# tinganchen/AlignQ

Hardware: AMD Instinct MI355X
Metric: images/sec (train step, CDF+ADMM) ResNet-20 8-bit (higher is better)
Workload: dtype f32; 1 GPU; resnet20 CIFAR-shape 3x32x32, 8W/8A CDF+ADMM full train step (cdf_alignment_admm/resnet-20-cifar-10), batch 128/GPU, HIP-graph replay, batch-norm folded into the site kernels, channels-last tensors, all Conv2d_Q convolutions on alignq_conv*_nhwc (exact-product bf16 MFMA); global_batch=128, parallelism=dp1

## Files before the change

alignq_amd/csrc/conv_kernels.hip:

```cpp
#include <hip/hip_runtime.h>
#include <stdint.h>
#include <stdlib.h>

#include "../../include/alignq.h"
#include "site_internal.h"
#include "store_forms.h"
#include "wgrad_reduce_body.h"

namespace {

using namespace alignq_wgr;

typedef __bf16 bf16x8 __attribute__((ext_vector_type(8)));
typedef __bf16 bf16x4 __attribute__((ext_vector_type(4)));
typedef float f32x4 __attribute__((ext_vector_type(4)));
typedef short s16x4 __attribute__((ext_vector_type(4)));

#ifdef ALIGNQ_STAMPS
__device__ unsigned long long g_conv_stamps[64];
__device__ unsigned long long g_conv_blk[2][4096];
#define STAMP(on, i)                                                          \
  do {                                                                        \
    if ((on) && threadIdx.x == 0) g_conv_stamps[i] = wall_clock64();          \
  } while (0)
// ... 477 lines not shown
  if (bn_part) {
    float* red = reinterpret_cast<float*>(lds);
#define ROW_SHR_ADD(V, CTRL) V += __builtin_bit_cast(float, __builtin_amdgcn_update_dpp(0, __builtin_bit_cast(int, V), CTRL, 0xf, 0xf, false))
#pragma unroll
    for (int e = 0; e < 4; e++) {
      ROW_SHR_ADD(bs[e], 0x111); ROW_SHR_ADD(bs[e], 0x112); ROW_SHR_ADD(bs[e], 0x114); ROW_SHR_ADD(bs[e], 0x118);
      ROW_SHR_ADD(bq[e], 0x111); ROW_SHR_ADD(bq[e], 0x112); ROW_SHR_ADD(bq[e], 0x114); ROW_SHR_ADD(bq[e], 0x118);
    }
#undef ROW_SHR_ADD
    __syncthreads();
    if ((lane & 15) == 15) {
#pragma unroll
      for (int e = 0; e < 4; e++) {
        red[(wv * 16 + 4 * q + e) * 2] = bs[e];
        red[(wv * 16 + 4 * q + e) * 2 + 1] = bq[e];
      }
    }
    __syncthreads();
    if (tid < COUT) {
      const int cg = tid / 16, cl = tid % 16;
      float s0 = 0.f, s1 = 0.f;
#pragma unroll
      for (int ppi = 0; ppi < NPP; ppi++) {
        s0 += red[((ppi * NCG + cg) * 16 + cl) * 2];
        s1 += red[((ppi * NCG + cg) * 16 + cl) * 2 + 1];
      }
      bn_part[((int64_t)tid * n_wg + block) * 2] = s0;
      bn_part[((int64_t)tid * n_wg + block) * 2 + 1] = s1;
    }
  }
}

template <int CIN, int COUT, int WDI, int KS, int S, int PT, bool IMG = false>
__global__ __launch_bounds__(256) void convgen_fwd_kernel(const float* __restrict__ x, const float* __restrict__ w,
                                                          float* __restrict__ y, int H, int total_rows, float nlev,
                                                          float* __restrict__ bn_part) {
  __shared__ __attribute__((aligned(16))) __bf16 lds[3 * ConvGen<CIN, COUT, WDI, KS, S, PT>::ARR];
  convgen_fwd_body<CIN, COUT, WDI, KS, S, PT, IMG>(x, w, y, H, total_rows, nlev, bn_part, lds, blockIdx.x, gridDim.x);
}

template <int CIN, int COUT, int WDI, int PT3, int PT1, bool IMG = false>
__global__ __launch_bounds__(256) void transition_fwd_kernel(const float* __restrict__ x, const float* __restrict__ w3,
                                                             const float* __restrict__ w1, float* __restrict__ y3,
                                                             float* __restrict__ y1, int H, int total_rows, float nlev,
                                                             float* __restrict__ part3, float* __restrict__ part1, int n3) {
  constexpr int A3 = ConvGen<CIN, COUT, WDI, 3, 2, PT3>::ARR, A1 = ConvGen<CIN, COUT, WDI, 1, 2, PT1>::ARR;
  __shared__ __attribute__((aligned(16))) __bf16 lds[3 * (A3 > A1 ? A3 : A1)];
  if ((int)blockIdx.x < n3)
    convgen_fwd_body<CIN, COUT, WDI, 3, 2, PT3, IMG>(x, w3, y3, H, total_rows, nlev, part3, lds, blockIdx.x, n3);
  else
    convgen_fwd_body<CIN, COUT, WDI, 1, 2, PT1, IMG>(x, w1, y1, H, total_rows, nlev, part1, lds, blockIdx.x - n3,
                                                     (int)gridDim.x - n3);
}

template <int CIN, int COUT, int WDI, int KS, int PT, bool WITH1, bool IMG = false>
__device__ __forceinline__ void dgrad_s2_body(const float* __restrict__ dy, const float* __restrict__ w,
                                              float* __restrict__ dx, int H, int total_rows, float nlev,
                                              const float* __restrict__ add, BnLazy lazy, __bf16* lds, int block,
                                              const float* __restrict__ dy1 = nullptr, const float* __restrict__ w1 = nullptr,
                                              BnLazy lazy1 = BnLazy{nullptr, nullptr, nullptr, nullptr}) {
  static_assert(!WITH1 || KS == 3, "the second source is the 1x1 shortcut of a 3x3 transition");
  constexpr int P = KS == 3 ? 1 : 0;
  constexpr int WDO = WDI / 2, TR = PT / WDI;
  constexpr int DROWS = TR / 2 + P, DCOLS = WDO + P;
  constexpr int CP = COUT + 8;
  constexpr int NPIX3 = DROWS * DCOLS + 1;
  constexpr int NPIX1 = WITH1 ? (TR / 2) * WDO : 0;
  constexpr int NPIX = NPIX3 + NPIX1;
  constexpr int ARR = NPIX * CP;
  constexpr int NT = KS * KS + (WITH1 ? 1 : 0);
  constexpr int NS = (NT * COUT + 31) / 32;
  constexpr int NCG = CIN / 16, NPP = 4 / NCG, NG = PT / 16;
  __bf16* Xhi = lds;
  __bf16* Xmi = lds + ARR;
  __bf16* Xlo = lds + 2 * ARR;
  const int tid = threadIdx.x, lane = tid & 63, wv = tid >> 6;
  const int row0 = block * TR;
  const int Ho = H / 2;
  const int orow0 = (row0 / H) * Ho + (row0 % H) / 2;
  const int oimg_hi = (row0 / H + 1) * Ho;
  {
    constexpr int C4 = COUT / 4;
    constexpr int N4 = NPIX3 * C4;
    constexpr int NIT = (N4 + 255) / 256;
    constexpr int M4 = NPIX1 * C4;
    constexpr int NI1 = WITH1 ? (M4 + 255) / 256 : 1;
    float4 v[NIT], zz[NIT], v1[NI1], z1[NI1];
#pragma unroll
    for (int it = 0; it < NIT; it++) {
      const int i = tid + 256 * it;
      const int c4 = i % C4, pix = i / C4;
      const int lr = pix / DCOLS, col = pix % DCOLS;
      const int grow = orow0 + lr;
      const bool ok = i < N4 && pix < DROWS * DCOLS && col < WDO && grow < oimg_hi;
      const int64_t off = ok ? ((int64_t)grow * WDO + col) * COUT + 4 * c4 : 0;
      v[it] = *reinterpret_cast<const float4*>(dy + off);
      if (lazy.z) zz[it] = *reinterpret_cast<const float4*>(lazy.z + off);
      if (!ok) v[it] = make_float4(0.f, 0.f, 0.f, 0.f);
    }
    if constexpr (WITH1) {
#pragma unroll
      for (int it = 0; it < NI1; it++) {
        const int i = tid + 256 * it;
        const int64_t off = i < M4 ? ((int64_t)orow0 * WDO) * COUT + 4 * (int64_t)i : 0;
        v1[it] = *reinterpret_cast<const float4*>(dy1 + off);
        if (lazy1.z) z1[it] = *reinterpret_cast<const float4*>(lazy1.z + off);
      }
    }
    const int c4t = tid % C4;
    if (lazy.z) {
      const float4 a4 = *reinterpret_cast<const float4*>(lazy.ab + 4 * c4t);
      const float4 m4 = *reinterpret_cast<const float4*>(lazy.save + 4 * c4t);
      const float4 i4 = *reinterpret_cast<const float4*>(lazy.save + COUT + 4 * c4t);
      float4 k0, k1;
      if (lazy.part) {
        __shared__ __attribute__((aligned(16))) float kt[2 * COUT];
        bn_totals_lds<COUT>(lazy, kt, block == 0);
        k0 = *reinterpret_cast<const float4*>(kt + 4 * c4t);
        k1 = *reinterpret_cast<const float4*>(kt + COUT + 4 * c4t);
      } else {
        k0 = *reinterpret_cast<const float4*>(lazy.ktot + 4 * c4t);
        k1 = *reinterpret_cast<const float4*>(lazy.ktot + COUT + 4 * c4t);
      }
#pragma unroll
      for (int it = 0; it < NIT; it++) {
        const int i = tid + 256 * it;
        const int pix = i / C4;
        const int lr = pix / DCOLS, col = pix % DCOLS;
        const bool ok = i < N4 && pix < DROWS * DCOLS && col < WDO && orow0 + lr < oimg_hi;
        if (ok) v[it] = bn_lazy4(v[it], zz[it], a4, m4, i4, k0, k1);
      }
    }
    if constexpr (WITH1) {
      if (lazy1.z) {
        const float4 a4 = *reinterpret_cast<const float4*>(lazy1.ab + 4 * c4t);
        const float4 m4 = *reinterpret_cast<const float4*>(lazy1.save + 4 * c4t);
        const float4 i4 = *reinterpret_cast<const float4*>(lazy1.save + COUT + 4 * c4t);
        float4 k0, k1;
        if (lazy1.part) {
          __shared__ __attribute__((aligned(16))) float kt1[2 * COUT];
          bn_totals_lds<COUT>(lazy1, kt1, block == 0);
          k0 = *reinterpret_cast<const float4*>(kt1 + 4 * c4t);
          k1 = *reinterpret_cast<const float4*>(kt1 + COUT + 4 * c4t);
        } else {
          k0 = *reinterpret_cast<const float4*>(lazy1.ktot + 4 * c4t);
          k1 = *reinterpret_cast<const float4*>(lazy1.ktot + COUT + 4 * c4t);
        }
#pragma unroll
        for (int it = 0; it < NI1; it++) {
          if (tid + 256 * it < M4) v1[it] = bn_lazy4(v1[it], z1[it], a4, m4, i4, k0, k1);
        }
      }
    }
#pragma unroll
    for (int it = 0; it < NIT + (WITH1 ? NI1 : 0); it++) {
      const bool second = it >= NIT;
      const int i = tid + 256 * (second ? it - NIT : it);
      if (i < (second ? M4 : N4)) {
        const int c4 = i % C4, pix = (second ? NPIX3 : 0) + i / C4;
        bf16x4 h4, m4, l4;
        const float4 src = second ? v1[second ? it - NIT : 0] : v[second ? 0 : it];
        const float vv[4] = {src.x, src.y, src.z, src.w};
#pragma unroll
        for (int e = 0; e < 4; e++) {
          const __bf16 hi = (__bf16)vv[e];
          const float r1 = vv[e] - (float)hi;
          const __bf16 mi = (__bf16)r1;
          h4[e] = hi; m4[e] = mi; l4[e] = (__bf16)(r1 - (float)mi);
        }
        const int o = pix * CP + 4 * c4;
        *reinterpret_cast<bf16x4*>(Xhi + o) = h4;
        *reinterpret_cast<bf16x4*>(Xmi + o) = m4;
        *reinterpret_cast<bf16x4*>(Xlo + o) = l4;
      }
    }
  }
  const int cig = wv % NCG, pp = wv / NCG;
  const int m = lane & 15, q = lane >> 4;
  bf16x8 ab[NS];
  if constexpr (IMG) {
    static_assert((KS * KS * COUT) % 32 == 0 && COUT % 32 == 0, "whole k steps per filter");
    constexpr int NS3 = KS * KS * COUT / 32;
    const bf16x8* __restrict__ wi = reinterpret_cast<const bf16x8*>(w) + (cig * NS3) * 64 + lane;
#pragma unroll
    for (int s = 0; s < NS3; s++) ab[s] = wi[s * 64];
    if constexpr (WITH1) {
      const bf16x8* __restrict__ wj = reinterpret_cast<const bf16x8*>(w1) + (cig * (NS - NS3)) * 64 + lane;
#pragma unroll
      for (int s = NS3; s < NS; s++) ab[s] = wj[(s - NS3) * 64];
    }
  } else {
#pragma unroll
    for (int s = 0; s < NS; s++) {
      const int k0 = 32 * s + 8 * q;
      const int tap = k0 / COUT, c0 = k0 % COUT;
#pragma unroll
      for (int j = 0; j < 8; j++) {
        float v = 0.f;
        if (tap < KS * KS) v = w[((int64_t)(c0 + j) * (KS * KS) + tap) * CIN + cig * 16 + m];
        else if (WITH1 && tap == KS * KS) v = w1[(int64_t)(c0 + j) * CIN + cig * 16 + m];
        ab[s][j] = (__bf16)rintf(v * nlev);
      }
    }
  }
  __syncthreads();
  for (int g = pp; g < NG; g += NPP) {
    const int p = g * 16 + (lane & 15);
    const int r = p / WDI, c = p % WDI;
    f32x4 acc = {0.f, 0.f, 0.f, 0.f};
#pragma unroll
    for (int s = 0; s < NS; s++) {
      const int k0 = 32 * s + 8 * q;
      const int tap = k0 / COUT, c0 = k0 % COUT;
      int pix = DROWS * DCOLS;
      if (tap < KS * KS) {
        const int ky = tap / KS, kx = tap % KS;
        const int a = r + P - ky, b = c + P - kx;
        if (a >= 0 && b >= 0 && !(a & 1) && !(b & 1)) pix = (a >> 1) * DCOLS + (b >> 1);
      } else if (WITH1 && tap == KS * KS) {
        if (!(r & 1) && !(c & 1)) pix = NPIX3 + (r >> 1) * WDO + (c >> 1);
      }
      const int o = pix * CP + c0;
      const bf16x8 bh = *reinterpret_cast<const bf16x8*>(Xhi + o);
      const bf16x8 bm = *reinterpret_cast<const bf16x8*>(Xmi + o);
      const bf16x8 bl = *reinterpret_cast<const bf16x8*>(Xlo + o);
      acc = __builtin_amdgcn_mfma_f32_16x16x32_bf16(ab[s], bl, acc, 0, 0, 0);
      acc = __builtin_amdgcn_mfma_f32_16x16x32_bf16(ab[s], bm, acc, 0, 0, 0);
      acc = __builtin_amdgcn_mfma_f32_16x16x32_bf16(ab[s], bh, acc, 0, 0, 0);
    }
    const int grow = row0 + r;
    if (grow < total_rows) {
      const int64_t o = ((int64_t)grow * WDI + c) * CIN + cig * 16 + 4 * q;
      float4 out = make_float4(acc[0] / nlev, acc[1] / nlev, acc[2] / nlev, acc[3] / nlev);
      if (add) {
        const float4 a4 = *reinterpret_cast<const float4*>(add + o);
        out.x += a4.x; out.y += a4.y; out.z += a4.z; out.w += a4.w;
      }
      alignq_store::st16<alignq_store::kConvOut>(dx + o, out);
    }
  }
}

template <int CIN, int COUT, int WDI, int KS, int PT, bool WITH1>
struct DgradS2Lds {
  static constexpr int P = KS == 3 ? 1 : 0, TR = PT / WDI;
  static constexpr int kBf16 = 3 * (((TR / 2 + P) * (WDI / 2 + P) + 1) + (WITH1 ? (TR / 2) * (WDI / 2) : 0)) * (COUT + 8);
};

template <int CIN, int COUT, int WDI, int KS, int PT, bool IMG = false>
__global__ __launch_bounds__(256) void dgrad_s2_kernel(const float* __restrict__ dy, const float* __restrict__ w,
                                                       float* __restrict__ dx, int H, int total_rows, float nlev,
                                                       const float* __restrict__ add, BnLazy lazy) {
  __shared__ __attribute__((aligned(16))) __bf16 lds[DgradS2Lds<CIN, COUT, WDI, KS, PT, false>::kBf16];
  dgrad_s2_body<CIN, COUT, WDI, KS, PT, false, IMG>(dy, w, dx, H, total_rows, nlev, add, lazy, lds, blockIdx.x);
}

template <int CIN, int COUT, int WDI, int KS, int PT>
int launch_dgrad_s2(const float* dy, const float* w, float* dx, int B, int H, float nlev, const float* add, BnLazy lazy,
                    hipStream_t st, bool img = false) {
  constexpr int TR = PT / WDI;
  static_assert(TR % 2 == 0, "even number of input rows per tile");
  if (H % TR) return ALIGNQ_EUNSUPPORTED;
  const int total_rows = B * H;
  if (img)
    hipLaunchKernelGGL((dgrad_s2_kernel<CIN, COUT, WDI, KS, PT, true>), total_rows / TR, 256, 0, st, dy, w, dx, H, total_rows, nlev,
                       add, lazy);
  else
    hipLaunchKernelGGL((dgrad_s2_kernel<CIN, COUT, WDI, KS, PT>), total_rows / TR, 256, 0, st, dy, w, dx, H, total_rows, nlev,
                       add, lazy);
  hipError_t e = hipGetLastError();
  return e == hipSuccess ? 0 : (int)e;
}

constexpr int kStemPT = 128;
__device__ __forceinline__ void stem_stage(const float* __restrict__ x, int H, int row0, __bf16* Chi, __bf16* Cmi, __bf16* Clo) {
  const int tid = threadIdx.x;
  const int pix = tid >> 1, half = tid & 1;
  const int r = pix / 32, c = pix % 32;
  const int grow = row0 + r;
  const int ih = grow % H;
  float v[16];
#pragma unroll
  for (int j = 0; j < 16; j++) {
    const int k = 16 * half + j;
    const int tap = k / 3, ci = k % 3;
    const int ky = tap / 3, kx = tap % 3;
    const int yy = ih + ky - 1, xx = c + kx - 1;
    const bool ok = k < 27 && yy >= 0 && yy < H && xx >= 0 && xx < 32;
    v[j] = x[ok ? ((int64_t)(grow + ky - 1) * 32 + xx) * 3 + ci : 0];
    if (!ok) v[j] = 0.f;
  }
  bf16x8 h[2], m[2], l[2];
#pragma unroll
  for (int j = 0; j < 16; j++) {
    const __bf16 hi = (__bf16)v[j];
    const float r1 = v[j] - (float)hi;
    const __bf16 mi = (__bf16)r1;
    h[j >> 3][j & 7] = hi; m[j >> 3][j & 7] = mi; l[j >> 3][j & 7] = (__bf16)(r1 - (float)mi);
  }
  const int o = pix * 32 + 16 * half;
  *reinterpret_cast<bf16x8*>(Chi + o) = h[0]; *reinterpret_cast<bf16x8*>(Chi + o + 8) = h[1];
  *reinterpret_cast<bf16x8*>(Cmi + o) = m[0]; *reinterpret_cast<bf16x8*>(Cmi + o + 8) = m[1];
  *reinterpret_cast<bf16x8*>(Clo + o) = l[0]; *reinterpret_cast<bf16x8*>(Clo + o + 8) = l[1];
// ... 169 lines not shown
template <int CIN, int COUT, int WDI, int KS, int S, int PT>
int launch_gen(const float* x, const float* w, float* y, int B, int H, float nlev, float* bn_part, hipStream_t st,
               bool img = false) {
  constexpr int TR = ConvGen<CIN, COUT, WDI, KS, S, PT>::TR;
  if (H % TR) return ALIGNQ_EUNSUPPORTED;
  const int total_rows = B * H;
  if (img)
    hipLaunchKernelGGL((convgen_fwd_kernel<CIN, COUT, WDI, KS, S, PT, true>), total_rows / TR, 256, 0, st, x, w, y, H, total_rows,
                       nlev, bn_part);
  else
    hipLaunchKernelGGL((convgen_fwd_kernel<CIN, COUT, WDI, KS, S, PT>), total_rows / TR, 256, 0, st, x, w, y, H, total_rows,
                       nlev, bn_part);
  hipError_t e = hipGetLastError();
  return e == hipSuccess ? 0 : (int)e;
}

template <int C, int WD, int PT>
int launch(const float* x, const float* w, float* y, int B, int H, int dgrad, float nlev, const float* add, float* bn_part,
           hipStream_t st, int xb = 0, float xlev = 1.0f, bool img = false) {
  constexpr int TR = PT / WD;
  const int total_rows = B * H;
  if (H % TR) return ALIGNQ_EUNSUPPORTED;
  const int grid = total_rows / TR;
  if (img) {
    if (dgrad) hipLaunchKernelGGL((conv3x3_nhwc_kernel<C, WD, PT, true, 0, true>), grid, 256, 0, st, x, w, y, H, total_rows, nlev, add, nullptr, 1.0f);
    else if (xb == 2) hipLaunchKernelGGL((conv3x3_nhwc_kernel<C, WD, PT, false, 2, true>), grid, 256, 0, st, x, w, y, H, total_rows, nlev, add, bn_part, xlev);
    else if (xb == 1) hipLaunchKernelGGL((conv3x3_nhwc_kernel<C, WD, PT, false, 1, true>), grid, 256, 0, st, x, w, y, H, total_rows, nlev, add, bn_part, xlev);
    else hipLaunchKernelGGL((conv3x3_nhwc_kernel<C, WD, PT, false, 0, true>), grid, 256, 0, st, x, w, y, H, total_rows, nlev, add, bn_part, xlev);
  } else if (dgrad) hipLaunchKernelGGL((conv3x3_nhwc_kernel<C, WD, PT, true, 0>), grid, 256, 0, st, x, w, y, H, total_rows, nlev, add, nullptr, 1.0f);
  else if (xb == 2) hipLaunchKernelGGL((conv3x3_nhwc_kernel<C, WD, PT, false, 2>), grid, 256, 0, st, x, w, y, H, total_rows, nlev, add, bn_part, xlev);
  else if (xb == 1) hipLaunchKernelGGL((conv3x3_nhwc_kernel<C, WD, PT, false, 1>), grid, 256, 0, st, x, w, y, H, total_rows, nlev, add, bn_part, xlev);
  else hipLaunchKernelGGL((conv3x3_nhwc_kernel<C, WD, PT, false, 0>), grid, 256, 0, st, x, w, y, H, total_rows, nlev, add, bn_part, xlev);
  hipError_t e = hipGetLastError();
  return e == hipSuccess ? 0 : (int)e;
}

typedef float f32x16 __attribute__((ext_vector_type(16)));

template <int CIN, int COUT, int WDI, int KS, int S, int PT>
struct WgradGeo {
  static constexpr int WDO = WDI / S, TR = PT / WDO, NT = KS * KS;
  static constexpr int CB = (CIN < COUT ? CIN : COUT) >= 32 ? 32 : 16;
  static constexpr int XROWS = KS == 3 ? TR * S + (S == 1 ? 2 : 1) : TR;
  static constexpr int LW = KS == 3 ? WDI + 2 : WDO;
  static constexpr int XA = XROWS * LW * CB;
  static constexpr int DA = PT * CB;
  static constexpr int kRed = 3 * NT * 4 * 64 * 4;
  static constexpr int kBytes = (3 * (XA + DA) * 2) > kRed ? (3 * (XA + DA) * 2) : kRed;
  static constexpr int kFloats = kBytes / 4;
};
template <int C, int WD, int PT>
struct WgradLds : WgradGeo<C, C, WD, 3, 1, PT> {};

template <int CIN, int COUT, int WDI, int KS, int S, int PT, int XB = 0>
__device__ __forceinline__ void wgrad_body(const float* __restrict__ x, const float* __restrict__ dy,
                                           float* __restrict__ slabs, int H, int n_tiles, float* lds_f, int bx, int gx,
                                           int by, BnLazy lazy = BnLazy{nullptr, nullptr, nullptr, nullptr}, float xlev = 1.0f) {
  constexpr int xb = XB;
  using G = WgradGeo<CIN, COUT, WDI, KS, S, PT>;
  constexpr int WDO = G::WDO, TR = G::TR, NT = G::NT, CB = G::CB, LW = G::LW, XA = G::XA, DA = G::DA, XROWS = G::XROWS;
  constexpr int NBLK = CIN / CB;
  constexpr int NSTEP = PT / 32;
  static_assert(WDO % 8 == 0 && PT % 32 == 0, "a lane group's 8 pixels lie in one output row");
  __bf16* lds = reinterpret_cast<__bf16*>(lds_f);
  __bf16* Xi[3] = {lds, lds + XA, lds + 2 * XA};
  __bf16* Di[3] = {lds + 3 * XA, lds + 3 * XA + DA, lds + 3 * XA + 2 * DA};
  const int tid = threadIdx.x, lane = tid & 63, wv = tid >> 6;
  const int bi = by / NBLK, bj = by % NBLK;
  const int cob = CB == 32 ? (wv >> 1) : 0, cib = CB == 32 ? (wv & 1) : 0;
  const int g = lane >> 4, q = (lane & 15) >> 2, pcol = 4 * (lane & 3);

  [[maybe_unused]] const bool st_on = bx == 0 && by == 0;
  STAMP(st_on, 16);
  f32x4 acc[NT];
#pragma unroll
  for (int t = 0; t < NT; t++) acc[t] = (f32x4){0.f, 0.f, 0.f, 0.f};

  constexpr int C4 = CB / 4;
  constexpr int N4 = XROWS * LW * C4;
  constexpr int M4 = PT * C4;
  constexpr int NIX = (N4 + 255) / 256, NID = (M4 + 255) / 256;
  f32x4 rx[NIX], rd[NID], rz[NID];
  const int per = (n_tiles + gx - 1) / gx;
  const int t_begin = bx * per, t_end = (t_begin + per < n_tiles) ? t_begin + per : n_tiles;
  int nxt = t_begin;
  if (nxt < t_end) {
    const int row0_ = nxt * TR;
    const int img_lo_ = (row0_ / H) * (H * S), img_hi_ = img_lo_ + H * S;
#pragma unroll
    for (int it = 0; it < NIX; it++) {
      const int i = tid + 256 * it;
      const int c4 = i % C4, col = (i / C4) % LW, lr = i / (C4 * LW);
      const int grow = KS == 3 ? row0_ * S - 1 + lr : (row0_ + lr) * S;
      const int gcol = KS == 3 ? col - 1 : col * S;
      const bool ok = i < N4 && gcol >= 0 && gcol < WDI && grow >= img_lo_ && grow < img_hi_;
      const int64_t off = ok ? ((int64_t)grow * WDI + gcol) * CIN + bj * CB + 4 * c4 : 0;
      rx[it] = fetch_act4<XB>(x, off);
      if (!ok) rx[it] = (f32x4){0.f, 0.f, 0.f, 0.f};
    }
#pragma unroll
    for (int it = 0; it < NID; it++) {
      const int i = tid + 256 * it;
      const int64_t off = i < M4 ? ((int64_t)row0_ * WDO + i / C4) * COUT + bi * CB + 4 * (i % C4) : 0;
      rd[it] = *reinterpret_cast<const f32x4*>(dy + off);
      if (lazy.z) rz[it] = *reinterpret_cast<const f32x4*>(lazy.z + off);
    }
  }
  f32x4 la = {0, 0, 0, 0}, lm = la, li = la, lk0 = la, lk1 = la;
  if (lazy.z) {
    const int cq = bi * CB + 4 * (tid % C4);
    la = *reinterpret_cast<const f32x4*>(lazy.ab + cq);
    lm = *reinterpret_cast<const f32x4*>(lazy.save + cq);
    li = *reinterpret_cast<const f32x4*>(lazy.save + COUT + cq);
    if (lazy.part) {
      __shared__ __attribute__((aligned(16))) float kt[2 * COUT];
      bn_totals_lds<COUT>(lazy, kt, false);
      lk0 = *reinterpret_cast<const f32x4*>(kt + cq);
      lk1 = *reinterpret_cast<const f32x4*>(kt + COUT + cq);
    } else {
      lk0 = *reinterpret_cast<const f32x4*>(lazy.ktot + cq);
      lk1 = *reinterpret_cast<const f32x4*>(lazy.ktot + COUT + cq);
    }
  }
  STAMP(st_on, 17);
  for (int tile = t_begin; tile < t_end; tile++) {
// ... 14 lines not shown
        }
        const int o = (lr * LW + col) * CB + 4 * c4;
        *reinterpret_cast<bf16x4*>(Xi[0] + o) = h4;
        *reinterpret_cast<bf16x4*>(Xi[1] + o) = m4;
        *reinterpret_cast<bf16x4*>(Xi[2] + o) = l4;
      }
    }
#pragma unroll
    for (int it = 0; it < NID; it++) {
      const int i = tid + 256 * it;
      if (i < M4) {
        bf16x4 h4, m4, l4;
        f32x4 dv = rd[it];
        if (lazy.z) dv = la * (dv - lk0 - (rz[it] - lm) * li * lk1);
#pragma unroll
        for (int e = 0; e < 4; e++) {
          const float v = dv[e];
          const __bf16 hi = (__bf16)v;
          const float r1 = v - (float)hi;
          const __bf16 mi = (__bf16)r1;
          h4[e] = hi; m4[e] = mi; l4[e] = (__bf16)(r1 - (float)mi);
        }
        const int o = (i / C4) * CB + 4 * (i % C4);
        *reinterpret_cast<bf16x4*>(Di[0] + o) = h4;
        *reinterpret_cast<bf16x4*>(Di[1] + o) = m4;
        *reinterpret_cast<bf16x4*>(Di[2] + o) = l4;
      }
    }
    __syncthreads();
    STAMP(st_on && tile - t_begin < 16, 18 + 2 * (tile - t_begin));
    nxt = tile + 1;
    if (nxt < t_end) {
      const int row0_ = nxt * TR;
      const int img_lo_ = (row0_ / H) * (H * S), img_hi_ = img_lo_ + H * S;
#pragma unroll
      for (int it = 0; it < NIX; it++) {
        const int i = tid + 256 * it;
        const int c4 = i % C4, col = (i / C4) % LW, lr = i / (C4 * LW);
        const int grow = KS == 3 ? row0_ * S - 1 + lr : (row0_ + lr) * S;
        const int gcol = KS == 3 ? col - 1 : col * S;
        const bool ok = i < N4 && gcol >= 0 && gcol < WDI && grow >= img_lo_ && grow < img_hi_;
        const int64_t off = ok ? ((int64_t)grow * WDI + gcol) * CIN + bj * CB + 4 * c4 : 0;
        rx[it] = fetch_act4<XB>(x, off);
        if (!ok) rx[it] = (f32x4){0.f, 0.f, 0.f, 0.f};
      }
#pragma unroll
      for (int it = 0; it < NID; it++) {
        const int i = tid + 256 * it;
        const int64_t off = i < M4 ? ((int64_t)row0_ * WDO + i / C4) * COUT + bi * CB + 4 * (i % C4) : 0;
        rd[it] = *reinterpret_cast<const f32x4*>(dy + off);
        if (lazy.z) rz[it] = *reinterpret_cast<const f32x4*>(lazy.z + off);
      }
    }
    for (int s = (CB == 16 ? wv : 0); s < NSTEP; s += (CB == 16 ? 4 : 1)) {
      const int p0 = 32 * s + 8 * g;
      const int r = p0 / WDO, c0 = p0 % WDO;
      bf16x8 a[3];
#pragma unroll
      for (int t = 0; t < 3; t++) {
        const __bf16* pa = Di[t] + (p0 + q) * CB + cob * 16 + pcol;
        a[t] = join8(tr_read(pa), tr_read(pa + 4 * CB));
      }
#pragma unroll
      for (int tap = 0; tap < NT; tap++) {
        const int ky = tap / KS, kx = tap % KS;
        bf16x8 b[3];
#pragma unroll
        for (int t = 0; t < 3; t++) {
          const __bf16* pb = Xi[t] + (KS == 3 ? ((r * S + ky) * LW + ((c0 + q) * S + kx)) : (r * LW + c0 + q)) * CB +
                             cib * 16 + pcol;
          b[t] = join8(tr_read(pb), tr_read(pb + 4 * (KS == 3 ? S : 1) * CB));
        }
        f32x4 v = acc[tap];
        v = __builtin_amdgcn_mfma_f32_16x16x32_bf16(a[1], b[1], v, 0, 0, 0);
        if (xb == 0) v = __builtin_amdgcn_mfma_f32_16x16x32_bf16(a[0], b[2], v, 0, 0, 0);
        v = __builtin_amdgcn_mfma_f32_16x16x32_bf16(a[2], b[0], v, 0, 0, 0);
        v = __builtin_amdgcn_mfma_f32_16x16x32_bf16(a[0], b[1], v, 0, 0, 0);
        v = __builtin_amdgcn_mfma_f32_16x16x32_bf16(a[1], b[0], v, 0, 0, 0);
        v = __builtin_amdgcn_mfma_f32_16x16x32_bf16(a[0], b[0], v, 0, 0, 0);
        acc[tap] = v;
      }
    }
    STAMP(st_on && tile - t_begin < 16, 19 + 2 * (tile - t_begin));
  }
  STAMP(st_on, 50);
  float* slab = slabs + (int64_t)bx * (NT * CIN * COUT);
  if (xb != 0) {
    const float inv = 1.0f / xlev;
#pragma unroll
    for (int t = 0; t < NT; t++) acc[t] = acc[t] * inv;
  }
  if (CB == 16) {
    float* red = lds_f;
    __syncthreads();
    if (wv > 0) {
#pragma unroll
      for (int t = 0; t < NT; t++)
#pragma unroll
        for (int e = 0; e < 4; e++) red[(((wv - 1) * NT + t) * 4 + e) * 64 + lane] = acc[t][e];
    }
    __syncthreads();
    if (wv == 0) {
#pragma unroll
      for (int t = 0; t < NT; t++) {
#pragma unroll
        for (int e = 0; e < 4; e++) {
          float v = acc[t][e];
#pragma unroll
          for (int w2 = 0; w2 < 3; w2++) v += red[((w2 * NT + t) * 4 + e) * 64 + lane];
          alignq_store::st4<alignq_store::kConvWgradSlab, true>(&slab[((int64_t)(bi * CB + 4 * (lane >> 4) + e) * NT + t) * CIN + bj * CB + (lane & 15)], v);
        }
      }
    }
  } else {
#pragma unroll
    for (int t = 0; t < NT; t++)
#pragma unroll
      for (int e = 0; e < 4; e++)
        alignq_store::st4<alignq_store::kConvWgradSlab, true>(&slab[((int64_t)(bi * CB + cob * 16 + 4 * (lane >> 4) + e) * NT + t) * CIN + bj * CB + cib * 16 + (lane & 15)], acc[t][e]);
  }
  STAMP(st_on, 51);
}

template <int C, int WD, int PT, int XB = 0>
__device__ __forceinline__ void wgrad3x3_body(const float* __restrict__ x, const float* __restrict__ dy,
                                              float* __restrict__ slabs, int H, int n_tiles, float* lds_f, int bx, int gx,
                                              int by, BnLazy lazy = BnLazy{nullptr, nullptr, nullptr, nullptr}, float xlev = 1.0f) {
  wgrad_body<C, C, WD, 3, 1, PT, XB>(x, dy, slabs, H, n_tiles, lds_f, bx, gx, by, lazy, xlev);
}

template <int CIN, int COUT, int WDI, int KS, int S, int PT>
__global__ __launch_bounds__(256) void wgradgen_kernel(const float* __restrict__ x, const float* __restrict__ dy,
                                                       float* __restrict__ slabs, int H, int n_tiles, BnLazy lazy) {
  __shared__ __attribute__((aligned(16))) float lds[WgradGeo<CIN, COUT, WDI, KS, S, PT>::kFloats];
  wgrad_body<CIN, COUT, WDI, KS, S, PT>(x, dy, slabs, H, n_tiles, lds, blockIdx.x, gridDim.x, blockIdx.y, lazy);
}

template <int C, int WD, int PT, int XB>
__global__ __launch_bounds__(256) void wgrad3x3_nhwc_kernel(const float* __restrict__ x, const float* __restrict__ dy,
                                                            float* __restrict__ slabs, int H, int n_tiles, float xlev) {
  __shared__ __attribute__((aligned(16))) float lds[WgradLds<C, WD, PT>::kFloats];
  wgrad3x3_body<C, WD, PT, XB>(x, dy, slabs, H, n_tiles, lds, blockIdx.x, gridDim.x, blockIdx.y,
                               BnLazy{nullptr, nullptr, nullptr, nullptr}, xlev);
}

template <int C, int WD, int PTD, int PTW, int XB, bool IMG = false>
__global__ __launch_bounds__(256) __attribute__((amdgpu_waves_per_eu(C == 16 ? 3 : 2, C == 16 ? 3 : 8)))
void conv3x3_bwd_kernel(const float* __restrict__ x, const float* __restrict__ dy,
                                                          const float* __restrict__ w, float* __restrict__ dx,
                                                          float* __restrict__ slabs, int H, int total_rows, float nlev,
                                                          int n_tiles_w, int splits, int nblk2,
                                                          const float* __restrict__ add, BnLazy lazy, float xlev, int dg_R,
                                                          RedFill fill, int n_dg) {
  constexpr int kBytesD = ConvLds<C, WD, PTD>::kBf16 * 2, kBytesW = WgradLds<C, WD, PTW>::kFloats * 4;
  static_assert(kBytesD >= 4096 || kBytesW >= 4096, "the filler role's 4 KB");
  __shared__ __attribute__((aligned(16))) unsigned char lds[kBytesD > kBytesW ? kBytesD : kBytesW];
  const int n_wg = splits * nblk2;
  BSTAMP(0);
  if ((int)blockIdx.x < n_wg) {
    wgrad3x3_body<C, WD, PTW, XB>(x, dy, slabs, H, n_tiles_w, reinterpret_cast<float*>(lds), blockIdx.x % splits, splits,
                                  blockIdx.x / splits, lazy, xlev);
  } else if ((int)blockIdx.x >= n_wg + n_dg) {
    const int fb = blockIdx.x - n_wg - n_dg;
    int it = 0;
    while (it + 1 < kFill && fb >= fill.blk0[it + 1]) it++;
    wgrad_reduce_body<256>(fill.slabs[it], fill.n_slabs[it], fill.n_elem[it], fill.dw[it], fb - fill.blk0[it],
                           reinterpret_cast<float*>(lds));
  } else {
    int m = blockIdx.x - n_wg;
    if (dg_R > 0) {
      const int i = (m / (8 * dg_R)) * 8 + (m & 7), r = (m >> 3) % dg_R;
      m = dg_R * i + r;
    }
    conv3x3_body<C, WD, PTD, true, 0, IMG>(dy, w, dx, H, total_rows, nlev, reinterpret_cast<__bf16*>(lds), m, add, nullptr, 0, lazy);
  }
  BSTAMP(1);
}

template <int CIN, int COUT, int WDI, int PTW3, int PTW1, int PTD, bool IMG = false>
__global__ __launch_bounds__(256) void transition_bwd_kernel(const float* __restrict__ x, const float* __restrict__ dy3,
                                                             const float* __restrict__ dy1, const float* __restrict__ w3,
                                                             const float* __restrict__ w1, float* __restrict__ dx,
                                                             float* __restrict__ slabs3, float* __restrict__ slabs1, int Ho,
                                                             int n_tiles3, int n_tiles1, int splits3, int splits1, int n_d,
                                                             float nlev, const float* __restrict__ add, BnLazy lazy3,
                                                             BnLazy lazy1, int dg_R) {
  using G3 = WgradGeo<CIN, COUT, WDI, 3, 2, PTW3>;
  using G1 = WgradGeo<CIN, COUT, WDI, 1, 2, PTW1>;
  constexpr int NBY = (COUT / G3::CB) * (CIN / G3::CB);
  static_assert(G3::CB == G1::CB, "same channel blocking");
  constexpr int kD = DgradS2Lds<CIN, COUT, WDI, 3, PTD, true>::kBf16 * 2;
  constexpr int kW = G3::kBytes > G1::kBytes ? G3::kBytes : G1::kBytes;
  __shared__ __attribute__((aligned(16))) unsigned char lds[kD > kW ? kD : kW];
  const int n_w3 = splits3 * NBY;
  const int b = blockIdx.x;
  if (b < n_d) {
    int m = b;
    if (dg_R > 0) {
      const int i = (m / (8 * dg_R)) * 8 + (m & 7), r = (m >> 3) % dg_R;
      m = dg_R * i + r;
    }
    dgrad_s2_body<CIN, COUT, WDI, 3, PTD, true, IMG>(dy3, w3, dx, 2 * Ho, 0x7fffffff, nlev, add, lazy3,
                                                     reinterpret_cast<__bf16*>(lds), m, dy1, w1, lazy1);
  } else if (b < n_d + n_w3) {
    const int c = b - n_d;
    wgrad_body<CIN, COUT, WDI, 3, 2, PTW3>(x, dy3, slabs3, Ho, n_tiles3, reinterpret_cast<float*>(lds), c % splits3, splits3,
                                           c / splits3, lazy3);
  } else {
    const int c = b - n_d - n_w3;
    wgrad_body<CIN, COUT, WDI, 1, 2, PTW1>(x, dy1, slabs1, Ho, n_tiles1, reinterpret_cast<float*>(lds), c % splits1, splits1,
                                           c / splits1, lazy1);
  }
}

__global__ __launch_bounds__(1024) void wgrad_reduce_kernel(const float* __restrict__ slabs, int n_slabs, int n_elem,
                                                            float* __restrict__ dw) {
  __shared__ __attribute__((aligned(16))) float part[4096];
  wgrad_reduce_body(slabs, n_slabs, n_elem, dw, blockIdx.x, part);
}

constexpr int kWgMulti = 32;
struct WgChunk {
  const float* slabs[kWgMulti];
  float* dw[kWgMulti];
  int n_slabs[kWgMulti];
  int n_elem[kWgMulti];
  int blk0[kWgMulti + 1];
};
__global__ __launch_bounds__(1024) void wgrad_reduce_multi_kernel(WgChunk c, int cnt) {
  __shared__ __attribute__((aligned(16))) float part[4096];
  int t = 0;
  while (t + 1 < cnt && (int)blockIdx.x >= c.blk0[t + 1]) t++;
  wgrad_reduce_body(c.slabs[t], c.n_slabs[t], c.n_elem[t], c.dw[t], (int)blockIdx.x - c.blk0[t], part);
}

template <int C, int WD, int PT>
int launch_wgrad(const float* x, const float* dy, float* dw, float* ws, int B, int H, int* n_slabs_out, hipStream_t st,
                 int xb = 0, float xlev = 1.0f) {
  constexpr int TR = PT / WD;
  if (H % TR) return ALIGNQ_EUNSUPPORTED;
  const int n_tiles = B * H / TR;
  constexpr int NB = (C >= 32 ? C / 32 : 1);
  int splits = 256 / (NB * NB);
  if (splits > n_tiles) splits = n_tiles;
  if (xb == 2) hipLaunchKernelGGL((wgrad3x3_nhwc_kernel<C, WD, PT, 2>), dim3(splits, NB * NB), 256, 0, st, x, dy, ws, H, n_tiles, xlev);
  else if (xb == 1) hipLaunchKernelGGL((wgrad3x3_nhwc_kernel<C, WD, PT, 1>), dim3(splits, NB * NB), 256, 0, st, x, dy, ws, H, n_tiles, xlev);
  else hipLaunchKernelGGL((wgrad3x3_nhwc_kernel<C, WD, PT, 0>), dim3(splits, NB * NB), 256, 0, st, x, dy, ws, H, n_tiles, xlev);
  hipError_t e = hipGetLastError();
  if (e != hipSuccess) return (int)e;
  if (n_slabs_out) { *n_slabs_out = splits; return 0; }
  const int n_elem = 9 * C * C;
  hipLaunchKernelGGL(wgrad_reduce_kernel, wgrad_reduce_blocks(splits, n_elem), 1024, 0, st, ws, splits, n_elem, dw);
  e = hipGetLastError();
  return e == hipSuccess ? 0 : (int)e;
}

template <int C, int WD, int PTD, int PTW>
int launch_bwd(const float* x, const float* dy, const float* w, float* dx, float* ws, int B, int H, float nlev,
               int* n_slabs_out, const float* add, BnLazy lazy, hipStream_t st, int xb, float xlev, const RedFill& fill,
               bool img) {
  constexpr int TRD = PTD / WD, TRW = PTW / WD;
  if (H % TRD || H % TRW) return ALIGNQ_EUNSUPPORTED;
  const int total_rows = B * H;
  const int n_tiles_w = total_rows / TRW;
  constexpr int NB = (C >= 32 ? C / 32 : 1);
// ... 299 lines not shown
  const int H = H_in / 2;
  if (img) wt = image_of(w_img, COUT, KS * KS, CIN, 0);
  if (CIN == 16 && KS == 3) return launch_gen<16, 32, 32, 3, 2, 64>(x, wt, y, B, H, nlev, bn_part, st, img);
  if (CIN == 16 && KS == 1) return launch_gen<16, 32, 32, 1, 2, 128>(x, wt, y, B, H, nlev, bn_part, st, img);
  if (CIN == 32 && KS == 3) return launch_gen<32, 64, 16, 3, 2, 32>(x, wt, y, B, H, nlev, bn_part, st, img);
  if (CIN == 32 && KS == 1) return launch_gen<32, 64, 16, 1, 2, 64>(x, wt, y, B, H, nlev, bn_part, st, img);
  return ALIGNQ_EUNSUPPORTED;
}
int alignq_conv_gen_nhwc_fwd(const float* x, const float* wt, float* y, int B, int H_in, int W_in, int CIN, int COUT, int KS,
                             int stride, int w_bit, float* bn_part, void* stream) {
  return conv_gen_nhwc_fwd(x, wt, nullptr, y, B, H_in, W_in, CIN, COUT, KS, stride, w_bit, bn_part, stream);
}
int alignq_conv_gen_nhwc_fwd_img(const float* x, const float* wt, const void* w_img, float* y, int B, int H_in, int W_in, int CIN,
                                 int COUT, int KS, int stride, int w_bit, float* bn_part, void* stream) {
  if (!w_img) return ALIGNQ_EINVAL;
  return conv_gen_nhwc_fwd(x, wt, w_img, y, B, H_in, W_in, CIN, COUT, KS, stride, w_bit, bn_part, stream);
}

size_t alignq_conv_gen_wgrad_ws_bytes(int CIN, int COUT, int KS) { return (size_t)256 * KS * KS * (size_t)CIN * COUT * sizeof(float); }
int alignq_conv_gen_nhwc_wgrad(const float* x, const float* dy, float* dw, void* ws, int B, int H_in, int W_in, int CIN,
                               int COUT, int KS, int stride, int* n_slabs_out, const float* bn_z, const float* bn_ab,
                               const float* bn_save, const float* bn_ktot, const float* bn_dx_part, void* stream) {
  if (!x || !dy || !ws || B < 1 || (!dw && !n_slabs_out)) return ALIGNQ_EINVAL;
  if (bn_z && (!bn_ab || !bn_save || (!bn_ktot && !bn_dx_part))) return ALIGNQ_EINVAL;
  BnLazy lazy{bn_z, bn_ab, bn_save, bn_ktot};
  if (!alignq_conv_gen_bn_parts(B, H_in, W_in, CIN, COUT, KS, stride)) return ALIGNQ_EUNSUPPORTED;
  if (int rc = lazy_parts(lazy, bn_dx_part, nullptr, nullptr, B, COUT, (H_in / 2) * (W_in / 2))) return rc;
  if ((reinterpret_cast<uintptr_t>(x) | reinterpret_cast<uintptr_t>(dy) | reinterpret_cast<uintptr_t>(dw)) & 15) return ALIGNQ_EUNSUPPORTED;
  hipStream_t st = (hipStream_t)stream;
  const int H = H_in / 2;
  if (CIN == 16 && KS == 3) return launch_wgradgen<16, 32, 32, 3, 2, 64>(x, dy, dw, (float*)ws, B, H, n_slabs_out, lazy, st);
  if (CIN == 16 && KS == 1) return launch_wgradgen<16, 32, 32, 1, 2, 128>(x, dy, dw, (float*)ws, B, H, n_slabs_out, lazy, st);
  if (CIN == 32 && KS == 3) return launch_wgradgen<32, 64, 16, 3, 2, 64>(x, dy, dw, (float*)ws, B, H, n_slabs_out, lazy, st);
  if (CIN == 32 && KS == 1) return launch_wgradgen<32, 64, 16, 1, 2, 64>(x, dy, dw, (float*)ws, B, H, n_slabs_out, lazy, st);
  return ALIGNQ_EUNSUPPORTED;
}

static int conv_gen_nhwc_dgrad(const float* dy, const float* wt, const void* w_img, float* dx, int B, int H_in, int W_in, int CIN,
                               int COUT, int KS, int stride, int w_bit, const float* add, const float* bn_z, const float* bn_ab,
                               const float* bn_save, const float* bn_ktot, const float* bn_dx_part, float* bn_dgamma,
                               float* bn_dbeta, void* stream) {
  if (!dy || !wt || !dx || B < 1) return ALIGNQ_EINVAL;
  if (reinterpret_cast<uintptr_t>(w_img) & 15) return ALIGNQ_EUNSUPPORTED;
  const bool img = w_img != nullptr;
  if (add && (reinterpret_cast<uintptr_t>(add) & 15)) return ALIGNQ_EUNSUPPORTED;
  if (bn_z && (!bn_ab || !bn_save || (!bn_ktot && !bn_dx_part))) return ALIGNQ_EINVAL;
  if (w_bit < 1 || w_bit > 8 || !alignq_conv_gen_bn_parts(B, H_in, W_in, CIN, COUT, KS, stride)) return ALIGNQ_EUNSUPPORTED;
  if ((reinterpret_cast<uintptr_t>(dy) | reinterpret_cast<uintptr_t>(wt) | reinterpret_cast<uintptr_t>(dx)) & 15) return ALIGNQ_EUNSUPPORTED;
  hipStream_t st = (hipStream_t)stream;
  const float nlev = (float)((1 << w_bit) - 1);
  BnLazy lazy{bn_z, bn_ab, bn_save, bn_ktot};
  if (int rc = lazy_parts(lazy, bn_dx_part, bn_dgamma, bn_dbeta, B, COUT, (H_in / 2) * (W_in / 2))) return rc;
  if (img) wt = image_of(w_img, COUT, KS * KS, CIN, 1);
  if (CIN == 16 && KS == 3) return launch_dgrad_s2<16, 32, 32, 3, 128>(dy, wt, dx, B, H_in, nlev, add, lazy, st, img);
  if (CIN == 16 && KS == 1) return launch_dgrad_s2<16, 32, 32, 1, 128>(dy, wt, dx, B, H_in, nlev, add, lazy, st, img);
  if (CIN == 32 && KS == 3) return launch_dgrad_s2<32, 64, 16, 3, 128>(dy, wt, dx, B, H_in, nlev, add, lazy, st, img);
  if (CIN == 32 && KS == 1) return launch_dgrad_s2<32, 64, 16, 1, 128>(dy, wt, dx, B, H_in, nlev, add, lazy, st, img);
  return ALIGNQ_EUNSUPPORTED;
}
int alignq_conv_gen_nhwc_dgrad(const float* dy, const float* wt, float* dx, int B, int H_in, int W_in, int CIN, int COUT, int KS,
                               int stride, int w_bit, const float* add, const float* bn_z, const float* bn_ab,
                               const float* bn_save, const float* bn_ktot, const float* bn_dx_part, float* bn_dgamma,
                               float* bn_dbeta, void* stream) {
  return conv_gen_nhwc_dgrad(dy, wt, nullptr, dx, B, H_in, W_in, CIN, COUT, KS, stride, w_bit, add, bn_z, bn_ab, bn_save, bn_ktot,
                             bn_dx_part, bn_dgamma, bn_dbeta, stream);
}
int alignq_conv_gen_nhwc_dgrad_img(const float* dy, const float* wt, const void* w_img, float* dx, int B, int H_in, int W_in,
                                   int CIN, int COUT, int KS, int stride, int w_bit, const float* add, const float* bn_z,
                                   const float* bn_ab, const float* bn_save, const float* bn_ktot, const float* bn_dx_part,
                                   float* bn_dgamma, float* bn_dbeta, void* stream) {
  if (!w_img) return ALIGNQ_EINVAL;
  return conv_gen_nhwc_dgrad(dy, wt, w_img, dx, B, H_in, W_in, CIN, COUT, KS, stride, w_bit, add, bn_z, bn_ab, bn_save, bn_ktot,
                             bn_dx_part, bn_dgamma, bn_dbeta, stream);
}

static int transition_nhwc_fwd(const float* x, const float* wt3, const float* wt1, const void* w_img3, const void* w_img1,
                               float* y3, float* y1, int B, int H_in, int W_in, int CIN, int COUT, int w_bit, float* bn_part3,
                               float* bn_part1, void* stream) {
  if (!x || !wt3 || !wt1 || !y3 || !y1 || B < 1 || !w_img3 != !w_img1) return ALIGNQ_EINVAL;
  if ((reinterpret_cast<uintptr_t>(w_img3) | reinterpret_cast<uintptr_t>(w_img1)) & 15) return ALIGNQ_EUNSUPPORTED;
  const bool img = w_img3 != nullptr;
  if (w_bit < 1 || w_bit > 8 || !alignq_conv_gen_bn_parts(B, H_in, W_in, CIN, COUT, 3, 2) ||
      !alignq_conv_gen_bn_parts(B, H_in, W_in, CIN, COUT, 1, 2))
    return ALIGNQ_EUNSUPPORTED;
  if ((reinterpret_cast<uintptr_t>(x) | reinterpret_cast<uintptr_t>(wt3) | reinterpret_cast<uintptr_t>(wt1) |
       reinterpret_cast<uintptr_t>(y3) | reinterpret_cast<uintptr_t>(y1)) & 15)
    return ALIGNQ_EUNSUPPORTED;
  hipStream_t st = (hipStream_t)stream;
  const float nlev = (float)((1 << w_bit) - 1);
  const int H = H_in / 2;
  if (img) { wt3 = image_of(w_img3, COUT, 9, CIN, 0); wt1 = image_of(w_img1, COUT, 1, CIN, 0); }
  if (CIN == 16) return launch_transition_fwd<16, 32, 32, 64, 128>(x, wt3, wt1, y3, y1, B, H, nlev, bn_part3, bn_part1, st, img);
  if (CIN == 32) return launch_transition_fwd<32, 64, 16, 32, 64>(x, wt3, wt1, y3, y1, B, H, nlev, bn_part3, bn_part1, st, img);
  return ALIGNQ_EUNSUPPORTED;
}
int alignq_transition_nhwc_fwd(const float* x, const float* wt3, const float* wt1, float* y3, float* y1, int B, int H_in,
                               int W_in, int CIN, int COUT, int w_bit, float* bn_part3, float* bn_part1, void* stream) {
  return transition_nhwc_fwd(x, wt3, wt1, nullptr, nullptr, y3, y1, B, H_in, W_in, CIN, COUT, w_bit, bn_part3, bn_part1, stream);
}
int alignq_transition_nhwc_fwd_img(const float* x, const float* wt3, const float* wt1, const void* w_img3, const void* w_img1,
                                   float* y3, float* y1, int B, int H_in, int W_in, int CIN, int COUT, int w_bit,
                                   float* bn_part3, float* bn_part1, void* stream) {
  if (!w_img3 || !w_img1) return ALIGNQ_EINVAL;
  return transition_nhwc_fwd(x, wt3, wt1, w_img3, w_img1, y3, y1, B, H_in, W_in, CIN, COUT, w_bit, bn_part3, bn_part1, stream);
}

static int transition_nhwc_bwd(const float* x, const float* dy3, const float* dy1, const float* wt3, const float* wt1,
                               const void* w_img3, const void* w_img1,
// ... 101 lines not shown
```

Before: 142,200 images/sec.

## Restructure stride-2 dgrad by parity class with pipelined LDS loads; pipeline wgrad taps

The stride-2 dgrad kernel now splits output pixels into the four parity classes. It uses a compile-time schedule that issues only the taps valid for each class, which removes the masked, wasted MFMAs, and it double-buffers the LDS fragment loads ahead of the MFMAs behind sched barriers. The wgrad body gains a software pipeline that keeps one or two taps of B fragments in flight across steps. The diff also adjusts waves-per-EU hints, doubles the dgrad pixel tile for CIN=16, and adds timing stamps. The price is higher register pressure from multiple accumulators and buffers, plus more complex scheduling code.

```diff
diff --git a/alignq_amd/csrc/conv_kernels.hip b/alignq_amd/csrc/conv_kernels.hip
--- a/alignq_amd/csrc/conv_kernels.hip
+++ b/alignq_amd/csrc/conv_kernels.hip
@@ -553,6 +553,33 @@
     convgen_fwd_body<CIN, COUT, WDI, 1, 2, PT1, IMG>(x, w1, y1, H, total_rows, nlev, part1, lds, blockIdx.x - n3,
                                                      (int)gridDim.x - n3);
 }
+
+template <int KS, int COUT, bool WITH1, int GW, int DCOLS>
+struct DgradS2Sched {
+  static constexpr int P = KS == 3 ? 1 : 0, SPT = COUT / 32, NS = (KS * KS + (WITH1 ? 1 : 0)) * SPT;
+  int n = 0;
+  int gi[GW * NS] = {}, s[GW * NS] = {}, off[GW * NS] = {}, c0[GW * NS] = {};
+  bool one[GW * NS] = {};
+  constexpr DgradS2Sched() {
+    for (int round = 0; round < NS; round++) {
+      for (int g = 0; g < GW; g++) {
+        const int rp = (g % 4) >> 1, cp = g & 1;
+        int live = 0;
+        for (int st = 0; st < NS; st++) {
+          const int tap = st / SPT, ky = tap / KS, kx = tap % KS;
+          const bool first = tap == KS * KS;
+          const bool ok = first ? (rp == 0 && cp == 0) : ((rp + P - ky) % 2 == 0 && (cp + P - kx) % 2 == 0);
+          if (!ok) continue;
+          if (live++ == round) {
+            gi[n] = g; s[n] = st; one[n] = first; c0[n] = 32 * (st % SPT);
+            off[n] = first ? 0 : ((rp + P - ky) / 2) * DCOLS + (cp + P - kx) / 2;
+            n++;
+          }
+        }
+      }
+    }
+  }
+};
 
 template <int CIN, int COUT, int WDI, int KS, int PT, bool WITH1, bool IMG = false>
 __device__ __forceinline__ void dgrad_s2_body(const float* __restrict__ dy, const float* __restrict__ w,
@@ -580,6 +607,7 @@
   const int Ho = H / 2;
   const int orow0 = (row0 / H) * Ho + (row0 % H) / 2;
   const int oimg_hi = (row0 / H + 1) * Ho;
+  STAMP(block == 0, 56);
   {
     constexpr int C4 = COUT / 4;
     constexpr int N4 = NPIX3 * C4;
@@ -608,6 +636,7 @@
         if (lazy1.z) z1[it] = *reinterpret_cast<const float4*>(lazy1.z + off);
       }
     }
+    STAMP(block == 0, 57);
     const int c4t = tid % C4;
     if (lazy.z) {
       const float4 a4 = *reinterpret_cast<const float4*>(lazy.ab + 4 * c4t);
@@ -676,9 +705,11 @@
       }
     }
   }
+  STAMP(block == 0, 58);
   const int cig = wv % NCG, pp = wv / NCG;
   const int m = lane & 15, q = lane >> 4;
   bf16x8 ab[NS];
+  static_assert(COUT % 32 == 0, "a k step lies inside one tap");
   if constexpr (IMG) {
     static_assert((KS * KS * COUT) % 32 == 0 && COUT % 32 == 0, "whole k steps per filter");
     constexpr int NS3 = KS * KS * COUT / 32;
@@ -704,35 +735,63 @@
       }
     }
   }
+  STAMP(block == 0, 59);
   __syncthreads();
-  for (int g = pp; g < NG; g += NPP) {
-    const int p = g * 16 + (lane & 15);
-    const int r = p / WDI, c = p % WDI;
-    f32x4 acc = {0.f, 0.f, 0.f, 0.f};
-#pragma unroll
-    for (int s = 0; s < NS; s++) {
-      const int k0 = 32 * s + 8 * q;
-      const int tap = k0 / COUT, c0 = k0 % COUT;
-      int pix = DROWS * DCOLS;
-      if (tap < KS * KS) {
-        const int ky = tap / KS, kx = tap % KS;
-        const int a = r + P - ky, b = c + P - kx;
-        if (a >= 0 && b >= 0 && !(a & 1) && !(b & 1)) pix = (a >> 1) * DCOLS + (b >> 1);
-      } else if (WITH1 && tap == KS * KS) {
-        if (!(r & 1) && !(c & 1)) pix = NPIX3 + (r >> 1) * WDO + (c >> 1);
-      }
-      const int o = pix * CP + c0;
-      const bf16x8 bh = *reinterpret_cast<const bf16x8*>(Xhi + o);
-      const bf16x8 bm = *reinterpret_cast<const bf16x8*>(Xmi + o);
-      const bf16x8 bl = *reinterpret_cast<const bf16x8*>(Xlo + o);
-      acc = __builtin_amdgcn_mfma_f32_16x16x32_bf16(ab[s], bl, acc, 0, 0, 0);
-      acc = __builtin_amdgcn_mfma_f32_16x16x32_bf16(ab[s], bm, acc, 0, 0, 0);
-      acc = __builtin_amdgcn_mfma_f32_16x16x32_bf16(ab[s], bh, acc, 0, 0, 0);
-    }
+  constexpr int GW = NG / NPP;
+  static_assert(NG % NPP == 0 && GW % 4 == 0, "every wave takes whole sets of the four parity classes");
+  using Sched = DgradS2Sched<KS, COUT, WITH1, GW, DCOLS>;
+  constexpr Sched sc{};
+  constexpr int NU = sc.n;
+  int bo[GW];
+  [[maybe_unused]] int bo1[GW];
+  f32x4 acc[GW];
+#pragma unroll
+  for (int gi = 0; gi < GW; gi++) {
+    const int idx = ((gi / 4) * NPP + pp) * 16 + (lane & 15);
+    bo[gi] = ((idx / WDO) * DCOLS + idx % WDO) * CP + 8 * q;
+    bo1[gi] = (NPIX3 + idx) * CP + 8 * q;
+    acc[gi] = (f32x4){0.f, 0.f, 0.f, 0.f};
+  }
+  {
+    constexpr int W = WITH1 ? 2 : 1;
+    bf16x8 bh[2][W], bm[2][W], bl[2][W];
+#pragma unroll
+    for (int u0 = -W; u0 < NU; u0 += W) {
+#pragma unroll
+      for (int d = 0; d < W; d++) {
+        const int u = u0 + W + d;
+        if (u < NU) {
+          const int o = (sc.one[u] ? bo1[sc.gi[u]] : bo[sc.gi[u]]) + sc.off[u] * CP + sc.c0[u];
+          bh[((u0 + W) / W) & 1][d] = *reinterpret_cast<const bf16x8*>(Xhi + o);
+          bm[((u0 + W) / W) & 1][d] = *reinterpret_cast<const bf16x8*>(Xmi + o);
+          bl[((u0 + W) / W) & 1][d] = *reinterpret_cast<const bf16x8*>(Xlo + o);
+        }
+      }
+      __builtin_amdgcn_sched_barrier(0);
+      if (u0 >= 0) {
+        const int sl = (u0 / W) & 1;
+        const bool same = W == 1 || (u0 + 1 < NU && sc.gi[u0] == sc.gi[u0 + 1]);
+#pragma unroll
+        for (int i = 0; i < 3 * W; i++) {
+          const int d = same ? i / 3 : i % W, t = same ? i % 3 : i / W;
+          const int u = u0 + d;
+          if (u < NU) {
+            const bf16x8 bt = t == 0 ? bl[sl][d] : (t == 1 ? bm[sl][d] : bh[sl][d]);
+            acc[sc.gi[u]] = __builtin_amdgcn_mfma_f32_16x16x32_bf16(ab[sc.s[u]], bt, acc[sc.gi[u]], 0, 0, 0);
+          }
+        }
+      }
+    }
+  }
+  STAMP(block == 0, 60);
+#pragma unroll
+  for (int gi = 0; gi < GW; gi++) {
+    const int idx = ((gi / 4) * NPP + pp) * 16 + (lane & 15);
+    const int r = 2 * (idx / WDO) + ((gi % 4) >> 1), c = 2 * (idx % WDO) + (gi & 1);
     const int grow = row0 + r;
     if (grow < total_rows) {
       const int64_t o = ((int64_t)grow * WDI + c) * CIN + cig * 16 + 4 * q;
-      float4 out = make_float4(acc[0] / nlev, acc[1] / nlev, acc[2] / nlev, acc[3] / nlev);
+      float4 out = make_float4(acc[gi][0] / nlev, acc[gi][1] / nlev, acc[gi][2] / nlev, acc[gi][3] / nlev);
       if (add) {
         const float4 a4 = *reinterpret_cast<const float4*>(add + o);
         out.x += a4.x; out.y += a4.y; out.z += a4.z; out.w += a4.w;
@@ -740,6 +799,7 @@
       alignq_store::st16<alignq_store::kConvOut>(dx + o, out);
     }
   }
+  STAMP(block == 0, 61);
 }
 
 template <int CIN, int COUT, int WDI, int KS, int PT, bool WITH1>
@@ -749,7 +809,7 @@
 };
 
 template <int CIN, int COUT, int WDI, int KS, int PT, bool IMG = false>
-__global__ __launch_bounds__(256) void dgrad_s2_kernel(const float* __restrict__ dy, const float* __restrict__ w,
+__global__ __launch_bounds__(256) __attribute__((amdgpu_waves_per_eu(4, 8))) void dgrad_s2_kernel(const float* __restrict__ dy, const float* __restrict__ w,
                                                        float* __restrict__ dx, int H, int total_rows, float nlev,
                                                        const float* __restrict__ add, BnLazy lazy) {
   __shared__ __attribute__((aligned(16))) __bf16 lds[DgradS2Lds<CIN, COUT, WDI, KS, PT, false>::kBf16];
@@ -1025,6 +1085,12 @@
 template <int C, int WD, int PT>
 struct WgradLds : WgradGeo<C, C, WD, 3, 1, PT> {};
 
+template <int CIN, int COUT, int NT, int S>
+constexpr int wgrad_taps_in_flight() {
+  if (CIN == 32 && COUT == 32) return 0;
+  return (NT > 1 && CIN == 16 && S == 2) ? 2 : 1;
+}
+
 template <int CIN, int COUT, int WDI, int KS, int S, int PT, int XB = 0>
 __device__ __forceinline__ void wgrad_body(const float* __restrict__ x, const float* __restrict__ dy,
                                            float* __restrict__ slabs, int H, int n_tiles, float* lds_f, int bx, int gx,
@@ -1043,7 +1109,7 @@
   const int cob = CB == 32 ? (wv >> 1) : 0, cib = CB == 32 ? (wv & 1) : 0;
   const int g = lane >> 4, q = (lane & 15) >> 2, pcol = 4 * (lane & 3);
 
-  [[maybe_unused]] const bool st_on = bx == 0 && by == 0;
+  [[maybe_unused]] const bool st_on = bx == 0 && by == 0 && KS == 3;
   STAMP(st_on, 16);
   f32x4 acc[NT];
 #pragma unroll
@@ -1164,33 +1230,54 @@
         if (lazy.z) rz[it] = *reinterpret_cast<const f32x4*>(lazy.z + off);
       }
     }
-    for (int s = (CB == 16 ? wv : 0); s < NSTEP; s += (CB == 16 ? 4 : 1)) {
-      const int p0 = 32 * s + 8 * g;
-      const int r = p0 / WDO, c0 = p0 % WDO;
-      bf16x8 a[3];
-#pragma unroll
-      for (int t = 0; t < 3; t++) {
-        const __bf16* pa = Di[t] + (p0 + q) * CB + cob * 16 + pcol;
-        a[t] = join8(tr_read(pa), tr_read(pa + 4 * CB));
-      }
-#pragma unroll
-      for (int tap = 0; tap < NT; tap++) {
-        const int ky = tap / KS, kx = tap % KS;
-        bf16x8 b[3];
-#pragma unroll
-        for (int t = 0; t < 3; t++) {
-          const __bf16* pb = Xi[t] + (KS == 3 ? ((r * S + ky) * LW + ((c0 + q) * S + kx)) : (r * LW + c0 + q)) * CB +
-                             cib * 16 + pcol;
-          b[t] = join8(tr_read(pb), tr_read(pb + 4 * (KS == 3 ? S : 1) * CB));
+    constexpr int TF = wgrad_taps_in_flight<CIN, COUT, NT, S>();
+    constexpr int SJ = (CB == 16 || CIN == 64 || TF == 0) ? 1 : NSTEP;
+    constexpr int U = SJ * NT;
+    constexpr int TD = TF == 0 ? 1 : TF;
+    static_assert(NT == 1 || NT > TD, "units computed together belong to different accumulators");
+    constexpr int AH = (TF == 0 || (CIN == 64 && xb == 0)) ? 0 : TD;
+    for (int sb = (CB == 16 ? wv : 0); sb < NSTEP; sb += (CB == 16 ? 4 : SJ)) {
+      bf16x8 a[2][3], b[2][TD][3];
+#pragma unroll
+      for (int u0 = -AH; u0 < U; u0 += TD) {
+#pragma unroll
+        for (int d = 0; d < TD; d++) {
+          const int u = u0 + AH + d;
+          if (u < U) {
+            const int j = u / NT, tap = u % NT, ky = tap / KS, kx = tap % KS;
+            const int p0 = 32 * (sb + j) + 8 * g;
+            const int r = p0 / WDO, c0 = p0 % WDO;
+            if (tap == 0) {
+#pragma unroll
+              for (int t = 0; t < 3; t++) {
+                const __bf16* pa = Di[t] + (p0 + q) * CB + cob * 16 + pcol;
+                a[j & 1][t] = join8(tr_read(pa), tr_read(pa + 4 * CB));
+              }
+            }
+#pragma unroll
+            for (int t = 0; t < (xb == 0 ? 3 : 2); t++) {
+              const __bf16* pb = Xi[t] + (KS == 3 ? ((r * S + ky) * LW + ((c0 + q) * S + kx)) : (r * LW + c0 + q)) * CB +
+                                 cib * 16 + pcol;
+              b[((u0 + AH) / TD) & 1][d][t] = join8(tr_read(pb), tr_read(pb + 4 * (KS == 3 ? S : 1) * CB));
+            }
+          }
         }
-        f32x4 v = acc[tap];
-        v = __builtin_amdgcn_mfma_f32_16x16x32_bf16(a[1], b[1], v, 0, 0, 0);
-        if (xb == 0) v = __builtin_amdgcn_mfma_f32_16x16x32_bf16(a[0], b[2], v, 0, 0, 0);
-        v = __builtin_amdgcn_mfma_f32_16x16x32_bf16(a[2], b[0], v, 0, 0, 0);
-        v = __builtin_amdgcn_mfma_f32_16x16x32_bf16(a[0], b[1], v, 0, 0, 0);
-        v = __builtin_amdgcn_mfma_f32_16x16x32_bf16(a[1], b[0], v, 0, 0, 0);
-        v = __builtin_amdgcn_mfma_f32_16x16x32_bf16(a[0], b[0], v, 0, 0, 0);
-        acc[tap] = v;
+        if (TF != 0) __builtin_amdgcn_sched_barrier(0);
+        if (u0 >= 0) {
+          constexpr int kTA[6] = {1, 0, 2, 0, 1, 0}, kTB[6] = {1, 2, 0, 1, 0, 0};
+#pragma unroll
+          for (int pr = 0; pr < 6; pr++) {
+            if (xb != 0 && kTB[pr] == 2) continue;
+#pragma unroll
+            for (int d = 0; d < TD; d++) {
+              const int u = u0 + d;
+              if (u < U) {
+                const int j = u / NT, tap = u % NT;
+                acc[tap] = __builtin_amdgcn_mfma_f32_16x16x32_bf16(a[j & 1][kTA[pr]], b[(u0 / TD) & 1][d][kTB[pr]], acc[tap], 0, 0, 0);
+              }
+            }
+          }
+        }
       }
     }
     STAMP(st_on && tile - t_begin < 16, 19 + 2 * (tile - t_begin));
@@ -1249,7 +1336,7 @@
 }
 
 template <int C, int WD, int PT, int XB>
-__global__ __launch_bounds__(256) void wgrad3x3_nhwc_kernel(const float* __restrict__ x, const float* __restrict__ dy,
+__global__ __launch_bounds__(256) __attribute__((amdgpu_waves_per_eu(C == 32 ? 2 : 3, 8))) void wgrad3x3_nhwc_kernel(const float* __restrict__ x, const float* __restrict__ dy,
                                                             float* __restrict__ slabs, int H, int n_tiles, float xlev) {
   __shared__ __attribute__((aligned(16))) float lds[WgradLds<C, WD, PT>::kFloats];
   wgrad3x3_body<C, WD, PT, XB>(x, dy, slabs, H, n_tiles, lds, blockIdx.x, gridDim.x, blockIdx.y,
@@ -1257,7 +1344,7 @@
 }
 
 template <int C, int WD, int PTD, int PTW, int XB, bool IMG = false>
-__global__ __launch_bounds__(256) __attribute__((amdgpu_waves_per_eu(C == 16 ? 3 : 2, C == 16 ? 3 : 8)))
+__global__ __launch_bounds__(256) __attribute__((amdgpu_waves_per_eu(C == 32 ? 2 : 3, C == 16 ? 3 : 8)))
 void conv3x3_bwd_kernel(const float* __restrict__ x, const float* __restrict__ dy,
                                                           const float* __restrict__ w, float* __restrict__ dx,
                                                           float* __restrict__ slabs, int H, int total_rows, float nlev,
@@ -1306,6 +1393,7 @@
   __shared__ __attribute__((aligned(16))) unsigned char lds[kD > kW ? kD : kW];
   const int n_w3 = splits3 * NBY;
   const int b = blockIdx.x;
+  BSTAMP(0);
   if (b < n_d) {
     int m = b;
     if (dg_R > 0) {
@@ -1323,6 +1411,7 @@
     wgrad_body<CIN, COUT, WDI, 1, 2, PTW1>(x, dy1, slabs1, Ho, n_tiles1, reinterpret_cast<float*>(lds), c % splits1, splits1,
                                            c / splits1, lazy1);
   }
+  BSTAMP(1);
 }
 
 __global__ __launch_bounds__(1024) void wgrad_reduce_kernel(const float* __restrict__ slabs, int n_slabs, int n_elem,
@@ -1728,8 +1817,8 @@
   BnLazy lazy{bn_z, bn_ab, bn_save, bn_ktot};
   if (int rc = lazy_parts(lazy, bn_dx_part, bn_dgamma, bn_dbeta, B, COUT, (H_in / 2) * (W_in / 2))) return rc;
   if (img) wt = image_of(w_img, COUT, KS * KS, CIN, 1);
-  if (CIN == 16 && KS == 3) return launch_dgrad_s2<16, 32, 32, 3, 128>(dy, wt, dx, B, H_in, nlev, add, lazy, st, img);
-  if (CIN == 16 && KS == 1) return launch_dgrad_s2<16, 32, 32, 1, 128>(dy, wt, dx, B, H_in, nlev, add, lazy, st, img);
+  if (CIN == 16 && KS == 3) return launch_dgrad_s2<16, 32, 32, 3, 256>(dy, wt, dx, B, H_in, nlev, add, lazy, st, img);
+  if (CIN == 16 && KS == 1) return launch_dgrad_s2<16, 32, 32, 1, 256>(dy, wt, dx, B, H_in, nlev, add, lazy, st, img);
   if (CIN == 32 && KS == 3) return launch_dgrad_s2<32, 64, 16, 3, 128>(dy, wt, dx, B, H_in, nlev, add, lazy, st, img);
   if (CIN == 32 && KS == 1) return launch_dgrad_s2<32, 64, 16, 1, 128>(dy, wt, dx, B, H_in, nlev, add, lazy, st, img);
   return ALIGNQ_EUNSUPPORTED;
```

Measured after the change: 143,800 images/sec (median of 5 runs). 1.01x the previous value.
